# mratsim/laser

Hardware: NVIDIA H100
Metric: sgemm_tflops_m8192_n8192_k8192 (higher is better)
Workload: dtype f32

## Files before the change

### laser_b200/csrc/capi.cu

```cuda
#include "../../include/laser_b200.h"

#include <cuda.h>
#include <cuda_runtime.h>
#include <cudaTypedefs.h>

#include <atomic>
#include <cstdarg>
#include <cstdio>
#include <cstdlib>
#include <cstring>
#include <map>
#include <mutex>
#include <string>
#include <type_traits>
#include <utility>
#include <vector>

#include "gemm_simt.cuh"
#include "gemm_dmma.cuh"
#include "layers.cuh"
#include "split.cuh"
#include "tc_launch.h"

namespace {
// ... 47 lines not shown
  int64_t depth, depth_stride;
  bool operator==(const MapKey &o) const {
    return base == o.base && inner == o.inner && outer == o.outer && stride == o.stride && esz == o.esz &&
           box_inner == o.box_inner && box_outer == o.box_outer && swz == o.swz && depth == o.depth &&
           depth_stride == o.depth_stride;
  }
};
struct MapCacheEntry {
  MapKey key;
  CUtensorMap map;
  bool valid = false;
};
constexpr int kMapCacheSize = 64;

constexpr int kSchedSlots = 256;

struct Ctx {
  MapCacheEntry map_cache[kMapCacheSize];
  int map_cache_next = 0;
  int raster_g = 0;
  bool splitk_enabled = true;
  bool f64_dmma = true;
  bool ring_attr_set = false, dmma_attr_set = false;
  int64_t panel_rows = 1024;
  bool panel_taper = false;
  int kc_faithful = 128;
  bool dyn_sched = true;
  bool pdl = true;
  int64_t batch_ws_bytes = static_cast<int64_t>(1024) << 20;
  bool profiling = false;
  std::vector<EventPair> prof;
  int dev = -1;
  int sm_count = 0;
  cudaStream_t stream = nullptr;
  cudaStream_t up = nullptr, down = nullptr;
  std::vector<cudaEvent_t> panel_ev;
  PFN_cuTensorMapEncodeTiled_v12000 encode = nullptr;
  Buffer ws[4];
  Buffer gather[2];
  Buffer stage[3];
  Buffer splitk;
  Buffer bpanels;
  Buffer layer_ws;
  Buffer tfilt;
  Buffer f16s;
  Buffer sched;
  int sched_next = 0;
  cudaEvent_t ws_free = nullptr;
  std::mutex mu;
  std::mutex host_mu;
  std::mutex tfilt_mu;
  std::atomic<bool> ready{false};
};

constexpr int kMaxDevices = 32;
Ctx g_ctx[kMaxDevices];
std::mutex g_ctx_mu;

int parse_f32_mode(const char *mode) {
  if (!mode) return kDefaultF32Mode;
  if (!strcmp(mode, "f16x3")) return LASER_B200_PATH_F16X3;
  else if (!strcmp(mode, "tf32x3")) return LASER_B200_PATH_TF32X3;
  else if (!strcmp(mode, "tf32x1")) return LASER_B200_PATH_TF32X1;
  else if (!strcmp(mode, "simt")) return LASER_B200_PATH_SIMT;
  return kDefaultF32Mode;
}

int get_ctx(Ctx **out) {
  int dev = 0;
  cudaError_t e = cudaGetDevice(&dev);
  if (e != cudaSuccess) {
    cudaGetLastError();
    return set_error(LASER_B200_ENODEVICE, "no CUDA device: %s", cudaGetErrorString(e));
  }
  if (dev < 0 || dev >= kMaxDevices) return set_error(LASER_B200_ENODEVICE, "device index %d", dev);
  Ctx &c = g_ctx[dev];
  if (!c.ready) {
    std::lock_guard<std::mutex> lk(g_ctx_mu);
    if (!c.ready) {
      cudaDeviceProp prop;
      CUDA_TRY(cudaGetDeviceProperties(&prop, dev));
      if (prop.major != 9 || prop.minor != 0)
        return set_error(LASER_B200_ENODEVICE,
                         "device %d is sm_%d%d; this library is built for sm_90a only (no fallback)",
                         dev, prop.major, prop.minor);
      c.dev = dev;
      c.sm_count = prop.multiProcessorCount;
      CUDA_TRY(cudaStreamCreateWithFlags(&c.stream, cudaStreamNonBlocking));
      CUDA_TRY(cudaStreamCreateWithFlags(&c.up, cudaStreamNonBlocking));
      CUDA_TRY(cudaStreamCreateWithFlags(&c.down, cudaStreamNonBlocking));
      CUDA_TRY(cudaEventCreateWithFlags(&c.ws_free, cudaEventDisableTiming));
      void *fn = nullptr;
      cudaDriverEntryPointQueryResult qres;
      CUDA_TRY(cudaGetDriverEntryPoint("cuTensorMapEncodeTiled", &fn, cudaEnableDefault, &qres));
      if (!fn || qres != cudaDriverEntryPointSuccess)
        return set_error(LASER_B200_ECUDA, "cuTensorMapEncodeTiled not available from the driver");
      c.encode = reinterpret_cast<PFN_cuTensorMapEncodeTiled_v12000>(fn);
      CUDA_TRY(cudaMalloc(&c.sched.ptr, kSchedSlots * 2 * sizeof(unsigned int)));
      c.sched.bytes = kSchedSlots * 2 * sizeof(unsigned int);
      CUDA_TRY(cudaMemset(c.sched.ptr, 0, c.sched.bytes));
      if (const char *kc = getenv("LASER_B200_KC")) {
        const int v = atoi(kc);
        if (v >= 32) c.kc_faithful = v;
      }
      if (const char *rg = getenv("LASER_B200_RASTER")) c.raster_g = atoi(rg);
      if (const char *sk = getenv("LASER_B200_SPLITK")) c.splitk_enabled = atoi(sk) != 0;
      if (const char *dm = getenv("LASER_B200_F64_DMMA")) c.f64_dmma = atoi(dm) != 0;
      if (const char *pt = getenv("LASER_B200_PANEL_TAPER")) c.panel_taper = atoi(pt) != 0;
      if (const char *ds = getenv("LASER_B200_DYNSCHED")) c.dyn_sched = atoi(ds) != 0;
      if (const char *pd = getenv("LASER_B200_PDL")) c.pdl = atoi(pd) != 0;
      if (const char *bw = getenv("LASER_B200_BATCH_WS_MB")) {
        const int64_t v = atoll(bw);
        if (v >= 1) c.batch_ws_bytes = v << 20;
      }
      if (const char *pr = getenv("LASER_B200_PANEL_ROWS")) {
        const int64_t v = atoll(pr) / 256 * 256;
        if (v >= 256) c.panel_rows = v;
      }
      if (g_f32_mode.load() < 0) g_f32_mode.store(parse_f32_mode(getenv("LASER_B200_F32_MODE")));
      c.ready = true;
// ... 484 lines not shown
  return path == LASER_B200_PATH_TF32X1 ? TC_TF32X1 : path == LASER_B200_PATH_TF32X3 ? TC_TF32X3 : TC_F16X3;
}
inline SplitMode split_mode(TcKind k) { return k == TC_TF32X3 ? SPLIT_TF32 : k == TC_F16X3 ? SPLIT_F16X2 : SPLIT_NONE; }

struct BatchArgs {
  int64_t batch, C, bias = 0;
};

template <typename OutT>
int tc_run(Ctx &c, TcKind kind, int64_t M, int64_t N, int64_t K, float alpha, const OperandMaps &ma,
           const OperandMaps &mb, float beta, OutT *C, int64_t rsC, int64_t csC, cudaStream_t s,
           const Epilogue &epi, const F16Scales *f16 = nullptr, bool after_prep = false, const BatchArgs *bat = nullptr,
           int64_t period_a = 1, int64_t period_b = 1) {
  TcLaunch l;
  l.a0 = ma.p0; l.a1 = ma.p1; l.b0 = mb.p0; l.b1 = mb.p1;
  l.a_mn = ma.mn_major; l.b_mn = mb.mn_major;
  l.pdl = c.pdl && after_prep;
  l.dev = c.dev; l.sm_count = c.sm_count; l.stream = s;
  TcParams &p = l.p;
  p.M = M; p.N = N; p.K = K; p.alpha = alpha; p.beta = beta;
  p.C = C; p.rsC = rsC; p.csC = csC; p.epi = epi;
  if (f16) { p.amax_a = f16->a; p.amax_b = f16->b; }
  if (bat) {
    l.batched = true;
    p.batch = static_cast<int>(bat->batch);
    p.period_a = static_cast<int>(period_a);
    p.period_b = static_cast<int>(period_b);
    p.bsC = bat->C;
    p.amax_bs_a = M;
    p.amax_bs_b = N;
    p.bias_bs = bat->bias;
  }
  const int npass = (kind == TC_TF32X3 || kind == TC_F16X3) ? 3 : 1;
  const TcPlanCfg cfg{c.kc_faithful, c.raster_g, c.splitk_enabled, c.sm_count};
  if (kind == TC_BF16 || kind == TC_F16X3) tc_plan<2, std::is_same<OutT, float>::value>(p, npass, cfg);
  else tc_plan<4, std::is_same<OutT, float>::value>(p, npass, cfg);
  if (c.dyn_sched) {
    p.sched = static_cast<unsigned int *>(c.sched.ptr) + 2 * c.sched_next;
    c.sched_next = (c.sched_next + 1) % kSchedSlots;
  }
  auto launch = [&](const TcLaunch &q) -> int {
    int e;
    switch (kind) {
      case TC_TF32X1: e = launch_tc_tf32x1(q); break;
      case TC_TF32X3: e = launch_tc_tf32x3(q); break;
      case TC_BF16: e = launch_tc_bf16(q); break;
      default: e = launch_tc_f16x3(q); break;
    }
    COUNT_LAUNCH();
    if (e != 0) {
      cudaGetLastError();
      return set_error(e == static_cast<int>(cudaErrorMemoryAllocation) ? LASER_B200_ENOMEM : LASER_B200_ECUDA,
                       "tensor-core kernel launch failed: %s", cudaGetErrorString(static_cast<cudaError_t>(e)));
    }
    CHECK_LAUNCH();
    return LASER_B200_OK;
  };
  ProfBracket prof;
  int rc = prof.open(c, s, 0);
  if (rc) return rc;
  if (p.k_splits > 1) {
    if constexpr (std::is_same<OutT, float>::value) {
      const int64_t ws_floats = tc_split_ws_floats(p);
      if ((rc = ensure(c.splitk, static_cast<size_t>(ws_floats) * sizeof(float)))) return rc;
      p.split_ws = static_cast<float *>(c.splitk.ptr);
      if ((rc = launch(l))) return rc;
      const int n_tail = p.num_m_blocks * p.num_n_blocks * p.batch - p.n_direct;
// ... 1297 lines not shown
```

### laser_b200/csrc/gemm_tc.cuh

```cuda
#pragma once

#include <type_traits>

#include "f16_scale.cuh"
#include "ptx.cuh"
#include "tc_params.h"

namespace lb200 {

#ifndef LB200_HOST_EMULATION
static __device__ __noinline__ float epi_act(float v, int act) {
#else
inline float epi_act(float v, int act) {
#endif
  if (act == 1) return fmaxf(v, 0.0f);
  if (act == 2) return tanhf(v);
  if (act == 3) return 1.0f / (1.0f + expf(-v));
  return v;
}

__device__ __forceinline__ float bf16_bits_to_f32(uint16_t h) {
  return __uint_as_float(static_cast<uint32_t>(h) << 16);
}
__device__ __forceinline__ uint16_t f32_to_bf16_bits(float f) {
  uint32_t u = __float_as_uint(f);
  if ((u & 0x7fffffffu) > 0x7f800000u) return static_cast<uint16_t>((u >> 16) | 0x40);
  u += 0x7fffu + ((u >> 16) & 1u);
  return static_cast<uint16_t>(u >> 16);
}

template <int ESZ, uint32_t FMT16, int NPASS, bool A_MN, bool B_MN, typename OutT, bool SCALED, bool BATCHED>
__global__ void __launch_bounds__(TC_THREADS, 1)
gemm_tc_kernel(const __grid_constant__ CUtensorMap mapA0, const __grid_constant__ CUtensorMap mapA1,
               const __grid_constant__ CUtensorMap mapB0, const __grid_constant__ CUtensorMap mapB1,
               const TcParams p) {
  static_assert(NPASS == 1 || NPASS == 3, "one pass, or the three passes of a two-piece product");
  static_assert(ESZ == 2 || (!A_MN && !B_MN), "wgmma reads tf32 operands K-major only (capi.cu transposes MN-major fp32)");
  using Cfg = TcCfg<NPASS>;
  constexpr int STAGES = Cfg::STAGES;
  constexpr int BLOCK_K = TC_ROW_BYTES / ESZ;
  const int sched_id = static_cast<int>(blockIdx.x);
  const int sched_stride = static_cast<int>(gridDim.x);

  LB200_DYN_SMEM(uint8_t, smem_raw);
  uint8_t *smem = reinterpret_cast<uint8_t *>((reinterpret_cast<uintptr_t>(smem_raw) + 1023) &
                                              ~static_cast<uintptr_t>(1023));
  uint64_t *bars = reinterpret_cast<uint64_t *>(smem + STAGES * Cfg::STAGE_BYTES);
  uint64_t *full_bar = bars;
  uint64_t *empty_bar = bars + STAGES;
  uint64_t *sched_full = bars + 2 * STAGES;
  uint64_t *sched_empty = sched_full + 1;
  int *sched_unit = reinterpret_cast<int *>(sched_empty + 1);

  const int warp_idx = threadIdx.x >> 5;
  const int lane = threadIdx.x & 31;
  const int tiles_pp = p.num_m_blocks * p.num_n_blocks;
  const int num_tiles = BATCHED ? tiles_pp * p.batch : tiles_pp;
  const int num_kb = static_cast<int>((p.K + BLOCK_K - 1) / BLOCK_K);
  const int num_units = p.n_direct + (num_tiles - p.n_direct) * p.k_splits;
  auto decode_unit = [&](int u, int &t, int &sp, int &kb_lo, int &kb_hi) {
    if (u < p.n_direct) {
      t = u; sp = -1; kb_lo = 0; kb_hi = num_kb;
    } else {
      const int v = u - p.n_direct;
      const int i = v / p.k_splits;
      t = p.n_direct + i;
      sp = v - i * p.k_splits;
      kb_lo = min(num_kb, sp * p.kb_per_split);
      kb_hi = min(num_kb, kb_lo + p.kb_per_split);
    }
  };
  constexpr int SCHED_CONSUMERS = 1 + TC_EPI_WARPS;
  auto next_unit = [&](uint32_t &ph) -> int {
    ptx::mbar_wait(sched_full, ph);
    const int u = *reinterpret_cast<volatile int *>(sched_unit);
    ptx::mbar_arrive(sched_empty);
    ph ^= 1u;
    return u;
  };

  if (threadIdx.x == 0) {
    ptx::prefetch_tensormap(&mapA0);
    ptx::prefetch_tensormap(&mapB0);
    if constexpr (NPASS == 3) {
      ptx::prefetch_tensormap(&mapA1);
      ptx::prefetch_tensormap(&mapB1);
    }
  }
  if (threadIdx.x == 32) {
    for (int i = 0; i < STAGES; ++i) {
      ptx::mbar_init(&full_bar[i], 1);
      ptx::mbar_init(&empty_bar[i], TC_EPI_WARPS);
    }
    ptx::mbar_init(sched_full, 1);
    ptx::mbar_init(sched_empty, SCHED_CONSUMERS);
    ptx::fence_barrier_init();
  }
  __syncthreads();
  ptx::griddep_wait();

  if (warp_idx < 4) {
    ptx::setmaxnreg_dec<TC_REGS_CTRL>();
    if (warp_idx == 3 && lane == 0) {
      uint32_t phase = 0;
      int next_static = sched_id;
      for (;;) {
        ptx::mbar_wait(sched_empty, phase ^ 1);
        int u;
        if (p.sched) {
          u = static_cast<int>(atomicAdd(p.sched, 1u));
        } else {
          u = next_static;
          next_static += sched_stride;
        }
        if (u >= num_units) u = -1;
        *reinterpret_cast<volatile int *>(sched_unit) = u;
        ptx::mbar_arrive(sched_full);
        phase ^= 1u;
        if (u < 0) {
          if (p.sched) {
            __threadfence();
            if (atomicAdd(p.sched + 1, 1u) == static_cast<unsigned int>(sched_stride - 1)) {
              p.sched[0] = 0u;
              p.sched[1] = 0u;
              __threadfence();
            }
          }
          break;
        }
      }
    } else if (warp_idx == 0 && lane == 0) {
      int stage = 0;
      uint32_t phase = 0, sched_phase = 0;
      constexpr int MN_ATOM = TC_ROW_BYTES / ESZ;
      constexpr int MN_BOX_BYTES = BLOCK_K * TC_ROW_BYTES;
      auto load_a = [&](uint8_t *dst, const CUtensorMap *m, uint64_t *bar, int m0, int k0, int z) {
        if constexpr (!A_MN) {
          if constexpr (BATCHED) ptx::tma_load_3d(dst, m, bar, k0, m0, z);
          else ptx::tma_load_2d(dst, m, bar, k0, m0);
        } else {
#pragma unroll
          for (int c = 0; c < TC_BLOCK_M / MN_ATOM; ++c) {
            if constexpr (BATCHED) ptx::tma_load_3d(dst + c * MN_BOX_BYTES, m, bar, m0 + c * MN_ATOM, k0, z);
            else ptx::tma_load_2d(dst + c * MN_BOX_BYTES, m, bar, m0 + c * MN_ATOM, k0);
          }
        }
      };
      auto load_b = [&](uint8_t *dst, const CUtensorMap *m, uint64_t *bar, int n0, int k0, int z) {
        if constexpr (!B_MN) {
          if constexpr (BATCHED) ptx::tma_load_3d(dst, m, bar, k0, n0, z);
          else ptx::tma_load_2d(dst, m, bar, k0, n0);
        } else {
#pragma unroll
          for (int c = 0; c < TC_BLOCK_N / MN_ATOM; ++c) {
            if constexpr (BATCHED) ptx::tma_load_3d(dst + c * MN_BOX_BYTES, m, bar, n0 + c * MN_ATOM, k0, z);
            else ptx::tma_load_2d(dst + c * MN_BOX_BYTES, m, bar, n0 + c * MN_ATOM, k0);
          }
        }
      };
      for (;;) {
        const int u = next_unit(sched_phase);
        if (u < 0) break;
        int t, sp, mb, nb, kb_lo, kb_hi;
        decode_unit(u, t, sp, kb_lo, kb_hi);
        int za = 0, zb = 0;
        if constexpr (BATCHED) {
          const int bz = t / tiles_pp;
          t -= bz * tiles_pp;
          za = bz % p.period_a;
          zb = bz % p.period_b;
        }
        tile_coords(t, p.num_m_blocks, p.num_n_blocks, p.raster_g, mb, nb);
        const int m0 = mb * TC_BLOCK_M;
        const int n0 = nb * TC_BLOCK_N;
        for (int kb = kb_lo; kb < kb_hi; ++kb) {
          ptx::mbar_wait(&empty_bar[stage], phase ^ 1);
          ptx::mbar_arrive_expect_tx(&full_bar[stage], Cfg::STAGE_BYTES);
          uint8_t *sa = smem + stage * Cfg::STAGE_BYTES;
          uint8_t *sb = sa + Cfg::A_STAGE_BYTES;
          const int k0 = kb * BLOCK_K;
          load_a(sa, &mapA0, &full_bar[stage], m0, k0, za);
          if constexpr (NPASS == 3) load_a(sa + TC_A_TILE_BYTES, &mapA1, &full_bar[stage], m0, k0, za);
          load_b(sb, &mapB0, &full_bar[stage], n0, k0, zb);
          if constexpr (NPASS == 3) load_b(sb + Cfg::B_TILE_BYTES, &mapB1, &full_bar[stage], n0, k0, zb);
          if (++stage == STAGES) { stage = 0; phase ^= 1; }
        }
      }
    }
  } else {
    ptx::setmaxnreg_inc<TC_REGS_EPI>();
    const int g = (warp_idx - 4) >> 2;
    const int wq = warp_idx & 3;
    const int lr = lane >> 2;
    const int lc = 2 * (lane & 3);
    constexpr int MMA_K = 32 / ESZ;
    constexpr int K_STEPS = BLOCK_K / MMA_K;
    constexpr int MN_BOX_BYTES = BLOCK_K * TC_ROW_BYTES;
    constexpr uint32_t A_WG_BYTES = 64 * TC_ROW_BYTES;
    int stage = 0;
    uint32_t phase = 0, sched_phase = 0;
    const bool vec_ok_c = (p.csC == 1) && ((p.rsC & 1) == 0) && ((reinterpret_cast<uintptr_t>(p.C) & (2 * sizeof(OutT) - 1)) == 0) &&
                          (!BATCHED || (p.bsC & 1) == 0);
    float acc[TC_ACC_REGS];
#pragma unroll
    for (int j = 0; j < TC_ACC_REGS; ++j) acc[j] = 0.0f;
    for (;;) {
      int u = 0;
      if (lane == 0) u = next_unit(sched_phase);
      u = __shfl_sync(0xffffffffu, u, 0);
      if (u < 0) break;
      int t, sp, mb, nb, kb_lo, kb_hi;
      decode_unit(u, t, sp, kb_lo, kb_hi);
      int bz = 0, za = 0, zb = 0;
      if constexpr (BATCHED) {
        bz = t / tiles_pp;
        za = bz % p.period_a;
        zb = bz % p.period_b;
        int tl = t - bz * tiles_pp;
        tile_coords(tl, p.num_m_blocks, p.num_n_blocks, p.raster_g, mb, nb);
      } else {
        tile_coords(t, p.num_m_blocks, p.num_n_blocks, p.raster_g, mb, nb);
      }
      const int num_blocks = (kb_hi - kb_lo + p.kb_per_block - 1) / p.kb_per_block;
      const int r_tile = 64 * g + 16 * wq + lr;
      const int64_t row0 = static_cast<int64_t>(mb) * TC_BLOCK_M + r_tile;
      const int64_t col0 = static_cast<int64_t>(nb) * TC_BLOCK_N + lc;
      const bool split_unit = sp >= 0;
      uint32_t amax_row[2] = {0u, 0u}, amax_col[2 * TC_BLOCK_N / 8];
      if constexpr (SCALED) {
#pragma unroll
        for (int h = 0; h < 2; ++h)
          if (row0 + 8 * h < p.M) amax_row[h] = p.amax_a[(BATCHED ? za * p.amax_bs_a : 0) + row0 + 8 * h];
#pragma unroll
        for (int j = 0; j < 2 * TC_BLOCK_N / 8; ++j) {
          const int64_t c = col0 + 8 * (j >> 1) + (j & 1);
          amax_col[j] = c < p.N ? p.amax_b[(BATCHED ? zb * p.amax_bs_b : 0) + c] : 0u;
        }
      }
      float run[TC_ACC_REGS];
#pragma unroll
      for (int j = 0; j < TC_ACC_REGS; ++j) run[j] = 0.0f;
      for (int blk = 0; blk < num_blocks; ++blk) {
        const int kb0 = kb_lo + blk * p.kb_per_block;
        const int kb1 = min(kb_hi, kb0 + p.kb_per_block);
        int prev_stage = -1;
        for (int kb = kb0; kb < kb1; ++kb) {
          ptx::mbar_wait(&full_bar[stage], phase);
          ptx::wgmma_fence();
          const uint32_t a_addr = ptx::smem_u32(smem + stage * Cfg::STAGE_BYTES) + g * A_WG_BYTES;
          const uint32_t b_addr = ptx::smem_u32(smem + stage * Cfg::STAGE_BYTES + Cfg::A_STAGE_BYTES);
#pragma unroll
          for (int pass = 0; pass < NPASS; ++pass) {
            const uint32_t a_tile = a_addr + ((NPASS == 3 && pass == 1) ? TC_A_TILE_BYTES : 0);
            const uint32_t b_tile = b_addr + ((NPASS == 3 && pass == 0) ? Cfg::B_TILE_BYTES : 0);
#pragma unroll
            for (int k = 0; k < K_STEPS; ++k) {
              const uint64_t ad = A_MN ? ptx::make_smem_desc(a_tile + k * MMA_K * TC_ROW_BYTES, MN_BOX_BYTES, 1024, ptx::kLayoutSw128)
                                       : ptx::make_smem_desc(a_tile + k * 32, 0, 1024, ptx::kLayoutSw128);
              const uint64_t bd = B_MN ? ptx::make_smem_desc(b_tile + k * MMA_K * TC_ROW_BYTES, MN_BOX_BYTES, 1024, ptx::kLayoutSw128)
                                       : ptx::make_smem_desc(b_tile + k * 32, 0, 1024, ptx::kLayoutSw128);
              const uint32_t accum = (kb == kb0 && pass == 0 && k == 0) ? 0u : 1u;
              if constexpr (ESZ == 4) ptx::wgmma_m64n128k8_tf32(acc, ad, bd, accum);
              else if constexpr (FMT16 == ptx::kFmtF16) ptx::wgmma_m64n128k16_f16<A_MN ? 1 : 0, B_MN ? 1 : 0>(acc, ad, bd, accum);
              else ptx::wgmma_m64n128k16_bf16<A_MN ? 1 : 0, B_MN ? 1 : 0>(acc, ad, bd, accum);
            }
          }
          ptx::wgmma_commit();
          ptx::wgmma_wait<1>();
          if (prev_stage >= 0 && lane == 0) ptx::mbar_arrive(&empty_bar[prev_stage]);
          prev_stage = stage;
          if (++stage == STAGES) { stage = 0; phase ^= 1; }
        }
        ptx::wgmma_wait<0>();
        ptx::wgmma_hold(acc);
        if (prev_stage >= 0 && lane == 0) ptx::mbar_arrive(&empty_bar[prev_stage]);
#pragma unroll
        for (int j = 0; j < TC_ACC_REGS; ++j) run[j] = __fadd_rn(run[j], acc[j]);
      }
      float alpha_r[2] = {split_unit ? 1.0f : p.alpha, split_unit ? 1.0f : p.alpha};
      if constexpr (SCALED) {
#pragma unroll
        for (int h = 0; h < 2; ++h) alpha_r[h] *= f16x2_unscale(amax_row[h]);
      }
      const float beta_u = split_unit ? 0.0f : p.beta;
      const bool has_epi = !split_unit && ((p.epi.bias != nullptr) || (p.epi.act != 0));
      float *ws_base = nullptr;
      if (split_unit) {
        const int64_t plane = static_cast<int64_t>(sp) * (num_tiles - p.n_direct) + (t - p.n_direct);
        ws_base = p.split_ws + (plane * TC_BLOCK_M + r_tile) * TC_BLOCK_N + lc;
      }
#pragma unroll
      for (int h = 0; h < 2; ++h) {
        const int64_t row = row0 + 8 * h;
        if (!split_unit && row >= p.M) continue;
        const float row_bias =
            (has_epi && p.epi.bias && p.epi.bias_per_row) ? p.epi.bias[(BATCHED ? za * p.bias_bs : 0) + row] : 0.0f;
        OutT *crow = split_unit ? nullptr : reinterpret_cast<OutT *>(p.C) + (BATCHED ? bz * p.bsC : 0) + row * p.rsC;
#pragma unroll
        for (int i = 0; i < TC_BLOCK_N / 8; ++i) {
          float v[2];
#pragma unroll
          for (int e = 0; e < 2; ++e) {
            v[e] = alpha_r[h] * run[4 * i + 2 * h + e];
            if constexpr (SCALED) v[e] *= f16x2_unscale(amax_col[2 * i + e]);
          }
          if (split_unit) {
            *reinterpret_cast<float2 *>(ws_base + 8 * h * TC_BLOCK_N + 8 * i) = make_float2(v[0], v[1]);
            continue;
          }
          const int64_t c = col0 + 8 * i;
          if (c >= p.N) continue;
          const bool pair_ok = vec_ok_c && c + 1 < p.N;
          OutT *dst = crow + c * p.csC;
          if (beta_u != 0.0f) {
            float o[2] = {0.0f, 0.0f};
            if constexpr (sizeof(OutT) == 4) {
              if (pair_ok) { const float2 w = *reinterpret_cast<const float2 *>(dst); o[0] = w.x; o[1] = w.y; }
              else { o[0] = dst[0]; if (c + 1 < p.N) o[1] = dst[p.csC]; }
            } else {
              o[0] = bf16_bits_to_f32(dst[0]);
              if (c + 1 < p.N) o[1] = bf16_bits_to_f32(dst[pair_ok ? 1 : p.csC]);
            }
#pragma unroll
            for (int e = 0; e < 2; ++e) v[e] = fmaf(beta_u, o[e], v[e]);
          }
          if (has_epi) {
#pragma unroll
            for (int e = 0; e < 2; ++e) {
              const float bv = (p.epi.bias && !p.epi.bias_per_row) ? (c + e < p.N ? p.epi.bias[c + e] : 0.0f) : row_bias;
              v[e] = epi_act(v[e] + bv, p.epi.act);
            }
          }
          if constexpr (sizeof(OutT) == 4) {
            if (pair_ok) *reinterpret_cast<float2 *>(dst) = make_float2(v[0], v[1]);
            else { dst[0] = v[0]; if (c + 1 < p.N) dst[p.csC] = v[1]; }
          } else {
            if (pair_ok) *reinterpret_cast<uint32_t *>(dst) = f32_to_bf16_bits(v[0]) | (static_cast<uint32_t>(f32_to_bf16_bits(v[1])) << 16);
            else { dst[0] = f32_to_bf16_bits(v[0]); if (c + 1 < p.N) dst[p.csC] = f32_to_bf16_bits(v[1]); }
          }
        }
      }
    }
  }

  __syncthreads();
}

}
```

### laser_b200/csrc/ptx.cuh

```cuda
#pragma once

#include <cuda.h>
#include <cuda_runtime.h>
#include <stdint.h>

#ifdef LB200_HOST_EMULATION
#include "ptx_emu.h"
#else

#define LB200_DYN_SMEM(T, name) extern __shared__ T name[]

namespace lb200 {
namespace ptx {

__device__ __forceinline__ uint32_t smem_u32(const void *p) {
  return static_cast<uint32_t>(__cvta_generic_to_shared(p));
}

__device__ __forceinline__ bool elect_one() {
  uint32_t pred = 0;
  asm volatile(
      "{\n\t"
      ".reg .pred P;\n\t"
      "elect.sync _|P, 0xffffffff;\n\t"
      "selp.u32 %0, 1, 0, P;\n\t"
      "}\n"
      : "=r"(pred));
  return pred != 0;
}

__device__ __forceinline__ void mbar_init(uint64_t *bar, uint32_t count) {
  asm volatile("mbarrier.init.shared::cta.b64 [%0], %1;" ::"r"(smem_u32(bar)), "r"(count));
}
__device__ __forceinline__ void fence_barrier_init() {
  asm volatile("fence.mbarrier_init.release.cluster;" ::: "memory");
}
__device__ __forceinline__ void fence_proxy_async_smem() {
  asm volatile("fence.proxy.async.shared::cta;" ::: "memory");
}
__device__ __forceinline__ void mbar_arrive_expect_tx(uint64_t *bar, uint32_t bytes) {
// ... 107 lines not shown
      "setp.ne.b32 p, %66, 0;\n\t"
      "wgmma.mma_async.sync.aligned.m64n128k16.f32.bf16.bf16 "
      "{%0, %1, %2, %3, %4, %5, %6, %7, %8, %9, %10, %11, %12, %13, %14, %15, %16, %17, %18, %19, %20, %21, %22, %23, %24, %25, %26, %27, %28, %29, %30, %31, %32, %33, %34, %35, %36, %37, %38, %39, %40, %41, %42, %43, %44, %45, %46, %47, %48, %49, %50, %51, %52, %53, %54, %55, %56, %57, %58, %59, %60, %61, %62, %63}, "
      "%64, %65, p, 1, 1, %67, %68;\n\t"
      "}\n"
      : "+f"(d[0]), "+f"(d[1]), "+f"(d[2]), "+f"(d[3]), "+f"(d[4]), "+f"(d[5]), "+f"(d[6]), "+f"(d[7]),
        "+f"(d[8]), "+f"(d[9]), "+f"(d[10]), "+f"(d[11]), "+f"(d[12]), "+f"(d[13]), "+f"(d[14]), "+f"(d[15]),
        "+f"(d[16]), "+f"(d[17]), "+f"(d[18]), "+f"(d[19]), "+f"(d[20]), "+f"(d[21]), "+f"(d[22]), "+f"(d[23]),
        "+f"(d[24]), "+f"(d[25]), "+f"(d[26]), "+f"(d[27]), "+f"(d[28]), "+f"(d[29]), "+f"(d[30]), "+f"(d[31]),
        "+f"(d[32]), "+f"(d[33]), "+f"(d[34]), "+f"(d[35]), "+f"(d[36]), "+f"(d[37]), "+f"(d[38]), "+f"(d[39]),
        "+f"(d[40]), "+f"(d[41]), "+f"(d[42]), "+f"(d[43]), "+f"(d[44]), "+f"(d[45]), "+f"(d[46]), "+f"(d[47]),
        "+f"(d[48]), "+f"(d[49]), "+f"(d[50]), "+f"(d[51]), "+f"(d[52]), "+f"(d[53]), "+f"(d[54]), "+f"(d[55]),
        "+f"(d[56]), "+f"(d[57]), "+f"(d[58]), "+f"(d[59]), "+f"(d[60]), "+f"(d[61]), "+f"(d[62]), "+f"(d[63])
      : "l"(a_desc), "l"(b_desc), "r"(scale_d), "n"(TA), "n"(TB));
}
__device__ __forceinline__ void wgmma_m64n128k8_tf32(float (&d)[64], uint64_t a_desc, uint64_t b_desc, uint32_t scale_d) {
  asm volatile(
      "{\n\t"
      ".reg .pred p;\n\t"
      "setp.ne.b32 p, %66, 0;\n\t"
      "wgmma.mma_async.sync.aligned.m64n128k8.f32.tf32.tf32 "
      "{%0, %1, %2, %3, %4, %5, %6, %7, %8, %9, %10, %11, %12, %13, %14, %15, %16, %17, %18, %19, %20, %21, %22, %23, %24, %25, %26, %27, %28, %29, %30, %31, %32, %33, %34, %35, %36, %37, %38, %39, %40, %41, %42, %43, %44, %45, %46, %47, %48, %49, %50, %51, %52, %53, %54, %55, %56, %57, %58, %59, %60, %61, %62, %63}, "
      "%64, %65, p, 1, 1;\n\t"
      "}\n"
      : "+f"(d[0]), "+f"(d[1]), "+f"(d[2]), "+f"(d[3]), "+f"(d[4]), "+f"(d[5]), "+f"(d[6]), "+f"(d[7]),
        "+f"(d[8]), "+f"(d[9]), "+f"(d[10]), "+f"(d[11]), "+f"(d[12]), "+f"(d[13]), "+f"(d[14]), "+f"(d[15]),
        "+f"(d[16]), "+f"(d[17]), "+f"(d[18]), "+f"(d[19]), "+f"(d[20]), "+f"(d[21]), "+f"(d[22]), "+f"(d[23]),
        "+f"(d[24]), "+f"(d[25]), "+f"(d[26]), "+f"(d[27]), "+f"(d[28]), "+f"(d[29]), "+f"(d[30]), "+f"(d[31]),
        "+f"(d[32]), "+f"(d[33]), "+f"(d[34]), "+f"(d[35]), "+f"(d[36]), "+f"(d[37]), "+f"(d[38]), "+f"(d[39]),
        "+f"(d[40]), "+f"(d[41]), "+f"(d[42]), "+f"(d[43]), "+f"(d[44]), "+f"(d[45]), "+f"(d[46]), "+f"(d[47]),
        "+f"(d[48]), "+f"(d[49]), "+f"(d[50]), "+f"(d[51]), "+f"(d[52]), "+f"(d[53]), "+f"(d[54]), "+f"(d[55]),
        "+f"(d[56]), "+f"(d[57]), "+f"(d[58]), "+f"(d[59]), "+f"(d[60]), "+f"(d[61]), "+f"(d[62]), "+f"(d[63])
      : "l"(a_desc), "l"(b_desc), "r"(scale_d));
}

__device__ __forceinline__ void griddep_wait() { asm volatile("griddepcontrol.wait;" ::: "memory"); }
__device__ __forceinline__ void griddep_launch_dependents() { asm volatile("griddepcontrol.launch_dependents;" ::: "memory"); }
constexpr uint32_t kLayoutSw128 = 1;
__device__ __forceinline__ uint64_t make_smem_desc(uint32_t smem_addr, uint32_t lbo_bytes, uint32_t sbo_bytes, uint32_t layout) {
  uint64_t d = 0;
  d |= static_cast<uint64_t>((smem_addr & 0x3FFFF) >> 4);
  d |= static_cast<uint64_t>((lbo_bytes >> 4) & 0x3FFF) << 16;
  d |= static_cast<uint64_t>((sbo_bytes >> 4) & 0x3FFF) << 32;
  d |= static_cast<uint64_t>(layout) << 62;
  return d;
}
constexpr uint32_t kFmtF16 = 0, kFmtBF16 = 1, kFmtTF32 = 2;

}
}

#endif
```

### laser_b200/csrc/tc_launch_impl.cuh

```cuda
#pragma once

#include <atomic>

#include "gemm_tc.cuh"
#include "tc_launch.h"

#ifndef LB200_LAUNCH_EX
#define LB200_LAUNCH_EX cudaLaunchKernelEx
#endif

namespace lb200 {

template <int ESZ, uint32_t FMT16, int NPASS, typename OutT, bool SCALED, bool A_MN, bool B_MN, bool BATCHED>
int launch_tc_one(const TcLaunch &l) {
  using Cfg = TcCfg<NPASS>;
  const int64_t units_total = tc_units(l.p);
  cudaLaunchConfig_t cfg{};
  cfg.gridDim = dim3(static_cast<int>(units_total < l.sm_count ? units_total : l.sm_count));
  cfg.blockDim = dim3(TC_THREADS);
  cfg.dynamicSmemBytes = Cfg::SMEM_BYTES;
  cfg.stream = l.stream;
  cudaLaunchAttribute attr[1];
  if (l.pdl) {
    attr[0].id = cudaLaunchAttributeProgrammaticStreamSerialization;
    attr[0].val.programmaticStreamSerializationAllowed = 1;
    cfg.attrs = attr;
    cfg.numAttrs = 1;
  }
  auto kfn = gemm_tc_kernel<ESZ, FMT16, NPASS, A_MN, B_MN, OutT, SCALED, BATCHED>;
  static std::atomic<uint32_t> attr_set{0};
  if (!(attr_set.load(std::memory_order_acquire) & (1u << l.dev))) {
    const cudaError_t e = cudaFuncSetAttribute(kfn, cudaFuncAttributeMaxDynamicSharedMemorySize, Cfg::SMEM_BYTES);
    if (e != cudaSuccess) return static_cast<int>(e);
    attr_set.fetch_or(1u << l.dev, std::memory_order_release);
  }
  return static_cast<int>(LB200_LAUNCH_EX(&cfg, kfn, l.a0, l.a1, l.b0, l.b1, l.p));
}

template <int ESZ, uint32_t FMT16, int NPASS, typename OutT, bool SCALED>
int launch_tc_family(const TcLaunch &l) {
  if constexpr (ESZ == 4) {
    if (l.a_mn || l.b_mn) return static_cast<int>(cudaErrorNotSupported);
    if (l.batched) return launch_tc_one<ESZ, FMT16, NPASS, OutT, SCALED, false, false, true>(l);
    return launch_tc_one<ESZ, FMT16, NPASS, OutT, SCALED, false, false, false>(l);
  }
#define LB200_MAJORS(BATCHED)                                                                                  \
  do {                                                                                                         \
    if (!l.a_mn && !l.b_mn) return launch_tc_one<ESZ, FMT16, NPASS, OutT, SCALED, false, false, BATCHED>(l);   \
    if (!l.a_mn && l.b_mn) return launch_tc_one<ESZ, FMT16, NPASS, OutT, SCALED, false, true, BATCHED>(l);     \
    if (l.a_mn && !l.b_mn) return launch_tc_one<ESZ, FMT16, NPASS, OutT, SCALED, true, false, BATCHED>(l);     \
    return launch_tc_one<ESZ, FMT16, NPASS, OutT, SCALED, true, true, BATCHED>(l);                             \
  } while (0)
  if constexpr (ESZ == 2) {
    if constexpr (SCALED) {
      if (l.batched) LB200_MAJORS(true);
    }
    if (l.batched) return static_cast<int>(cudaErrorNotSupported);
    LB200_MAJORS(false);
  }
#undef LB200_MAJORS
}

}
```

### laser_b200/csrc/tc_params.h

```cpp
#pragma once

#include <stdint.h>

#if defined(__CUDACC__) || defined(LB200_HOST_EMULATION)
#define LB200_HD __host__ __device__
#else
#define LB200_HD
#endif

namespace lb200 {

constexpr int TC_BLOCK_M = 128;
constexpr int TC_BLOCK_N = 128;
constexpr int TC_ROW_BYTES = 128;
constexpr int TC_A_TILE_BYTES = TC_BLOCK_M * TC_ROW_BYTES;
template <int NPASS> struct TcCfg {
  static constexpr int PIECES = (NPASS == 3) ? 2 : 1;
  static constexpr int B_TILE_BYTES = TC_BLOCK_N * TC_ROW_BYTES;
  static constexpr int A_STAGE_BYTES = PIECES * TC_A_TILE_BYTES;
  static constexpr int B_STAGE_BYTES = PIECES * B_TILE_BYTES;
  static constexpr int STAGE_BYTES = A_STAGE_BYTES + B_STAGE_BYTES;
#ifdef TC_STAGES_OVERRIDE
  static constexpr int STAGES = TC_STAGES_OVERRIDE;
#else
// ... 3 lines not shown
};
constexpr int TC_THREADS = 384;
constexpr int TC_EPI_THREADS = 256;
constexpr int TC_EPI_WARPS = TC_EPI_THREADS / 32;
constexpr int TC_ACC_REGS = 64 * TC_BLOCK_N / 128;
constexpr int TC_REGS_CTRL = 40;
constexpr int TC_REGS_EPI = 232;

struct Epilogue {
  const float *bias = nullptr;
  int bias_per_row = 0;
  int act = 0;
};
struct TcParams {
  int64_t M, N, K;
  float alpha, beta;
  void *C;
  int64_t rsC, csC;
  int kb_per_block;
  int raster_g;
  Epilogue epi;
  int n_direct;
  int k_splits;
  int kb_per_split;
  float *split_ws = nullptr;
  int num_m_blocks, num_n_blocks;
  const uint32_t *amax_a = nullptr, *amax_b = nullptr;
  unsigned int *sched = nullptr;
  int batch = 1;
  int period_a = 1, period_b = 1;
  int64_t bsC = 0;
  int64_t amax_bs_a = 0, amax_bs_b = 0;
  int64_t bias_bs = 0;
};

LB200_HD inline void tile_coords(int t, int num_m, int num_n, int G, int &mb, int &nb) {
  const int per_group = G * num_n;
  const int g = t / per_group;
  const int first_m = g * G;
  const int gsz = (G < num_m - first_m) ? G : (num_m - first_m);
  const int r = t - g * per_group;
  mb = first_m + r % gsz;
  nb = r / gsz;
}

struct TcPlanCfg {
  int kc_faithful;
  int raster_g;
  bool splitk_enabled;
  int sm_count;
  int tail_min_k = 2048;
};
template <int ESZ, bool OUT_F32>
inline void tc_plan(TcParams &p, int npass, const TcPlanCfg &cfg) {
  const int block_k = TC_ROW_BYTES / ESZ;
  const int num_kb = static_cast<int>((p.K + block_k - 1) / block_k);
  {
    const int kc = (npass == 3) ? cfg.kc_faithful : 0;
    p.kb_per_block = (kc > 0) ? (kc + block_k - 1) / block_k : num_kb;
    if (p.kb_per_block < 1) p.kb_per_block = 1;
    if (p.kb_per_block > num_kb) p.kb_per_block = num_kb;
  }
  p.raster_g = cfg.raster_g > 0 ? cfg.raster_g : 16;
  p.num_m_blocks = static_cast<int>((p.M + TC_BLOCK_M - 1) / TC_BLOCK_M);
  p.num_n_blocks = static_cast<int>((p.N + TC_BLOCK_N - 1) / TC_BLOCK_N);
  const int64_t tiles = static_cast<int64_t>(p.num_m_blocks) * p.num_n_blocks * p.batch;
  p.k_splits = 1;
  p.kb_per_split = num_kb;
  p.n_direct = static_cast<int>(tiles);
  p.split_ws = nullptr;
  const int units = cfg.sm_count;
  if constexpr (OUT_F32) {
    const int blocks = (num_kb + p.kb_per_block - 1) / p.kb_per_block;
    const int min_tiles = 512 / block_k;
    const int min_blocks = (min_tiles + p.kb_per_block - 1) / p.kb_per_block;
    const int max_s = blocks / min_blocks < 16 ? blocks / min_blocks : 16;
    const int64_t rem = tiles < units ? tiles : tiles % units;
    int S = rem > 0 ? static_cast<int>(units / rem) : 1;
    if (S > max_s) S = max_s;
    const bool worth = S >= 2 && (tiles < units || p.K >= cfg.tail_min_k);
    if (cfg.splitk_enabled && worth && units > 0) {
      const int blocks_per_split = (blocks + S - 1) / S;
      p.k_splits = (blocks + blocks_per_split - 1) / blocks_per_split;
      p.kb_per_split = blocks_per_split * p.kb_per_block;
      if (p.k_splits >= 2) p.n_direct = static_cast<int>(tiles - rem);
      else { p.k_splits = 1; p.kb_per_split = num_kb; }
    }
  }
}
inline int64_t tc_units(const TcParams &p) {
  const int64_t tiles = static_cast<int64_t>(p.num_m_blocks) * p.num_n_blocks * p.batch;
  return p.n_direct + (tiles - p.n_direct) * p.k_splits;
}
inline int64_t tc_split_ws_floats(const TcParams &p) {
  const int64_t tiles = static_cast<int64_t>(p.num_m_blocks) * p.num_n_blocks * p.batch;
  return (tiles - p.n_direct) * p.k_splits * TC_BLOCK_M * TC_BLOCK_N;
}

}
```

Measured before the change: 214.7.

## Pair CTAs in 2-CTA clusters and multicast shared B tiles via TMA

Launches the tensor-core GEMM kernel with clusters of two CTAs that work on vertically adjacent M tiles sharing the same N block. Each CTA loads the B tile for alternating k-blocks and multicasts it to both CTAs. The scheduler, stage releases and barriers become cluster-wide. This is meant to halve the L2/global traffic for B. In exchange it adds cross-CTA synchronisation, so one slow CTA stalls its partner, and the planner and unit decoding get more complex.

Result: slower. 125.5, median of 6 (-41.5%).

```diff
diff --git a/laser_b200/csrc/capi.cu b/laser_b200/csrc/capi.cu
--- a/laser_b200/csrc/capi.cu
+++ b/laser_b200/csrc/capi.cu
@@ -103,6 +103,7 @@
   std::vector<EventPair> prof;
   int dev = -1;
   int sm_count = 0;
+  bool cluster_launch = false;
   cudaStream_t stream = nullptr;
   cudaStream_t up = nullptr, down = nullptr;
   std::vector<cudaEvent_t> panel_ev;
@@ -157,6 +158,7 @@
                          dev, prop.major, prop.minor);
       c.dev = dev;
       c.sm_count = prop.multiProcessorCount;
+      c.cluster_launch = prop.clusterLaunch != 0;
       CUDA_TRY(cudaStreamCreateWithFlags(&c.stream, cudaStreamNonBlocking));
       CUDA_TRY(cudaStreamCreateWithFlags(&c.up, cudaStreamNonBlocking));
       CUDA_TRY(cudaStreamCreateWithFlags(&c.down, cudaStreamNonBlocking));
@@ -707,7 +709,8 @@
     p.bias_bs = bat->bias;
   }
   const int npass = (kind == TC_TF32X3 || kind == TC_F16X3) ? 3 : 1;
-  const TcPlanCfg cfg{c.kc_faithful, c.raster_g, c.splitk_enabled, c.sm_count};
+  TcPlanCfg cfg{c.kc_faithful, c.raster_g, c.splitk_enabled, c.sm_count};
+  cfg.pairs = c.cluster_launch;
   if (kind == TC_BF16 || kind == TC_F16X3) tc_plan<2, std::is_same<OutT, float>::value>(p, npass, cfg);
   else tc_plan<4, std::is_same<OutT, float>::value>(p, npass, cfg);
   if (c.dyn_sched) {
diff --git a/laser_b200/csrc/gemm_tc.cuh b/laser_b200/csrc/gemm_tc.cuh
--- a/laser_b200/csrc/gemm_tc.cuh
+++ b/laser_b200/csrc/gemm_tc.cuh
@@ -39,8 +39,10 @@
   using Cfg = TcCfg<NPASS>;
   constexpr int STAGES = Cfg::STAGES;
   constexpr int BLOCK_K = TC_ROW_BYTES / ESZ;
-  const int sched_id = static_cast<int>(blockIdx.x);
-  const int sched_stride = static_cast<int>(gridDim.x);
+  const int CL = p.cluster;
+  const uint32_t rank = CL > 1 ? ptx::cluster_ctarank() : 0u;
+  const int sched_id = static_cast<int>(blockIdx.x) / CL;
+  const int sched_stride = static_cast<int>(gridDim.x) / CL;
 
   LB200_DYN_SMEM(uint8_t, smem_raw);
   uint8_t *smem = reinterpret_cast<uint8_t *>((reinterpret_cast<uintptr_t>(smem_raw) + 1023) &
@@ -57,26 +59,53 @@
   const int tiles_pp = p.num_m_blocks * p.num_n_blocks;
   const int num_tiles = BATCHED ? tiles_pp * p.batch : tiles_pp;
   const int num_kb = static_cast<int>((p.K + BLOCK_K - 1) / BLOCK_K);
-  const int num_units = p.n_direct + (num_tiles - p.n_direct) * p.k_splits;
-  auto decode_unit = [&](int u, int &t, int &sp, int &kb_lo, int &kb_hi) {
-    if (u < p.n_direct) {
-      t = u; sp = -1; kb_lo = 0; kb_hi = num_kb;
+  const int unit_m = (p.num_m_blocks + CL - 1) / CL;
+  const int units_pp = unit_m * p.num_n_blocks;
+  const int num_unit_tiles = BATCHED ? units_pp * p.batch : units_pp;
+  const int num_units = p.n_direct_units + (num_unit_tiles - p.n_direct_units) * p.k_splits;
+  auto decode_unit = [&](int u, int &bz, int &mb, int &nb, int &t, int &sp, int &kb_lo, int &kb_hi) {
+    int q;
+    if (u < p.n_direct_units) {
+      q = u; sp = -1; kb_lo = 0; kb_hi = num_kb;
     } else {
-      const int v = u - p.n_direct;
+      const int v = u - p.n_direct_units;
       const int i = v / p.k_splits;
-      t = p.n_direct + i;
+      q = p.n_direct_units + i;
       sp = v - i * p.k_splits;
       kb_lo = min(num_kb, sp * p.kb_per_split);
       kb_hi = min(num_kb, kb_lo + p.kb_per_split);
     }
+    bz = BATCHED ? q / units_pp : 0;
+    tile_coords(q - bz * units_pp, unit_m, p.num_n_blocks, p.raster_g / CL, mb, nb);
+    if (CL == 1) {
+      t = q;
+    } else {
+      mb = CL * mb + static_cast<int>(rank);
+      t = mb < p.num_m_blocks ? bz * tiles_pp + tile_index(mb, nb, p.num_m_blocks, p.num_n_blocks, p.raster_g) : -1;
+    }
   };
   constexpr int SCHED_CONSUMERS = 1 + TC_EPI_WARPS;
   auto next_unit = [&](uint32_t &ph) -> int {
-    ptx::mbar_wait(sched_full, ph);
-    const int u = *reinterpret_cast<volatile int *>(sched_unit);
-    ptx::mbar_arrive(sched_empty);
+    int u;
+    if (CL == 1) {
+      ptx::mbar_wait(sched_full, ph);
+      u = *reinterpret_cast<volatile int *>(sched_unit);
+      ptx::mbar_arrive(sched_empty);
+    } else {
+      ptx::mbar_wait_cluster(sched_full, ph);
+      u = *reinterpret_cast<volatile int *>(sched_unit);
+      ptx::mbar_arrive_cluster(sched_empty, 0);
+    }
     ph ^= 1u;
     return u;
+  };
+  auto release_stage = [&](int s) {
+    if (CL == 1) {
+      ptx::mbar_arrive(&empty_bar[s]);
+    } else {
+      ptx::mbar_arrive_cluster(&empty_bar[s], 0);
+      ptx::mbar_arrive_cluster(&empty_bar[s], 1);
+    }
   };
 
   if (threadIdx.x == 0) {
@@ -90,18 +119,19 @@
   if (threadIdx.x == 32) {
     for (int i = 0; i < STAGES; ++i) {
       ptx::mbar_init(&full_bar[i], 1);
-      ptx::mbar_init(&empty_bar[i], TC_EPI_WARPS);
+      ptx::mbar_init(&empty_bar[i], CL * TC_EPI_WARPS);
     }
     ptx::mbar_init(sched_full, 1);
-    ptx::mbar_init(sched_empty, SCHED_CONSUMERS);
+    ptx::mbar_init(sched_empty, CL * SCHED_CONSUMERS);
     ptx::fence_barrier_init();
   }
-  __syncthreads();
+  if (CL > 1) ptx::cluster_sync();
+  else __syncthreads();
   ptx::griddep_wait();
 
   if (warp_idx < 4) {
     ptx::setmaxnreg_dec<TC_REGS_CTRL>();
-    if (warp_idx == 3 && lane == 0) {
+    if (warp_idx == 3 && lane == 0 && rank == 0) {
       uint32_t phase = 0;
       int next_static = sched_id;
       for (;;) {
@@ -114,8 +144,15 @@
           next_static += sched_stride;
         }
         if (u >= num_units) u = -1;
-        *reinterpret_cast<volatile int *>(sched_unit) = u;
-        ptx::mbar_arrive(sched_full);
+        if (CL == 1) {
+          *reinterpret_cast<volatile int *>(sched_unit) = u;
+          ptx::mbar_arrive(sched_full);
+        } else {
+          for (uint32_t r = 0; r < static_cast<uint32_t>(CL); ++r) {
+            ptx::st_shared_cluster_s32(sched_unit, r, u);
+            ptx::mbar_arrive_cluster(sched_full, r);
+          }
+        }
         phase ^= 1u;
         if (u < 0) {
           if (p.sched) {
@@ -147,30 +184,28 @@
         }
       };
       auto load_b = [&](uint8_t *dst, const CUtensorMap *m, uint64_t *bar, int n0, int k0, int z) {
+        auto box = [&](uint8_t *d, int c0, int c1) {
+          if (CL == 1) {
+            if constexpr (BATCHED) ptx::tma_load_3d(d, m, bar, c0, c1, z);
+            else ptx::tma_load_2d(d, m, bar, c0, c1);
+          } else {
+            if constexpr (BATCHED) ptx::tma_load_3d_multicast(d, m, bar, c0, c1, z, 0x3);
+            else ptx::tma_load_2d_multicast(d, m, bar, c0, c1, 0x3);
+          }
+        };
         if constexpr (!B_MN) {
-          if constexpr (BATCHED) ptx::tma_load_3d(dst, m, bar, k0, n0, z);
-          else ptx::tma_load_2d(dst, m, bar, k0, n0);
+          box(dst, k0, n0);
         } else {
 #pragma unroll
-          for (int c = 0; c < TC_BLOCK_N / MN_ATOM; ++c) {
-            if constexpr (BATCHED) ptx::tma_load_3d(dst + c * MN_BOX_BYTES, m, bar, n0 + c * MN_ATOM, k0, z);
-            else ptx::tma_load_2d(dst + c * MN_BOX_BYTES, m, bar, n0 + c * MN_ATOM, k0);
-          }
+          for (int c = 0; c < TC_BLOCK_N / MN_ATOM; ++c) box(dst + c * MN_BOX_BYTES, n0 + c * MN_ATOM, k0);
         }
       };
       for (;;) {
         const int u = next_unit(sched_phase);
         if (u < 0) break;
-        int t, sp, mb, nb, kb_lo, kb_hi;
-        decode_unit(u, t, sp, kb_lo, kb_hi);
-        int za = 0, zb = 0;
-        if constexpr (BATCHED) {
-          const int bz = t / tiles_pp;
-          t -= bz * tiles_pp;
-          za = bz % p.period_a;
-          zb = bz % p.period_b;
-        }
-        tile_coords(t, p.num_m_blocks, p.num_n_blocks, p.raster_g, mb, nb);
+        int bz, t, sp, mb, nb, kb_lo, kb_hi;
+        decode_unit(u, bz, mb, nb, t, sp, kb_lo, kb_hi);
+        const int za = BATCHED ? bz % p.period_a : 0, zb = BATCHED ? bz % p.period_b : 0;
         const int m0 = mb * TC_BLOCK_M;
         const int n0 = nb * TC_BLOCK_N;
         for (int kb = kb_lo; kb < kb_hi; ++kb) {
@@ -181,8 +216,10 @@
           const int k0 = kb * BLOCK_K;
           load_a(sa, &mapA0, &full_bar[stage], m0, k0, za);
           if constexpr (NPASS == 3) load_a(sa + TC_A_TILE_BYTES, &mapA1, &full_bar[stage], m0, k0, za);
-          load_b(sb, &mapB0, &full_bar[stage], n0, k0, zb);
-          if constexpr (NPASS == 3) load_b(sb + Cfg::B_TILE_BYTES, &mapB1, &full_bar[stage], n0, k0, zb);
+          if (CL == 1 || (kb & 1) == static_cast<int>(rank)) {
+            load_b(sb, &mapB0, &full_bar[stage], n0, k0, zb);
+            if constexpr (NPASS == 3) load_b(sb + Cfg::B_TILE_BYTES, &mapB1, &full_bar[stage], n0, k0, zb);
+          }
           if (++stage == STAGES) { stage = 0; phase ^= 1; }
         }
       }
@@ -209,18 +246,9 @@
       if (lane == 0) u = next_unit(sched_phase);
       u = __shfl_sync(0xffffffffu, u, 0);
       if (u < 0) break;
-      int t, sp, mb, nb, kb_lo, kb_hi;
-      decode_unit(u, t, sp, kb_lo, kb_hi);
-      int bz = 0, za = 0, zb = 0;
-      if constexpr (BATCHED) {
-        bz = t / tiles_pp;
-        za = bz % p.period_a;
-        zb = bz % p.period_b;
-        int tl = t - bz * tiles_pp;
-        tile_coords(tl, p.num_m_blocks, p.num_n_blocks, p.raster_g, mb, nb);
-      } else {
-        tile_coords(t, p.num_m_blocks, p.num_n_blocks, p.raster_g, mb, nb);
-      }
+      int bz, t, sp, mb, nb, kb_lo, kb_hi;
+      decode_unit(u, bz, mb, nb, t, sp, kb_lo, kb_hi);
+      const int za = BATCHED ? bz % p.period_a : 0, zb = BATCHED ? bz % p.period_b : 0;
       const int num_blocks = (kb_hi - kb_lo + p.kb_per_block - 1) / p.kb_per_block;
       const int r_tile = 64 * g + 16 * wq + lr;
       const int64_t row0 = static_cast<int64_t>(mb) * TC_BLOCK_M + r_tile;
@@ -267,13 +295,13 @@
           }
           ptx::wgmma_commit();
           ptx::wgmma_wait<1>();
-          if (prev_stage >= 0 && lane == 0) ptx::mbar_arrive(&empty_bar[prev_stage]);
+          if (prev_stage >= 0 && lane == 0) release_stage(prev_stage);
           prev_stage = stage;
           if (++stage == STAGES) { stage = 0; phase ^= 1; }
         }
         ptx::wgmma_wait<0>();
         ptx::wgmma_hold(acc);
-        if (prev_stage >= 0 && lane == 0) ptx::mbar_arrive(&empty_bar[prev_stage]);
+        if (prev_stage >= 0 && lane == 0) release_stage(prev_stage);
 #pragma unroll
         for (int j = 0; j < TC_ACC_REGS; ++j) run[j] = __fadd_rn(run[j], acc[j]);
       }
@@ -284,6 +312,7 @@
       }
       const float beta_u = split_unit ? 0.0f : p.beta;
       const bool has_epi = !split_unit && ((p.epi.bias != nullptr) || (p.epi.act != 0));
+      if (t < 0) continue;
       float *ws_base = nullptr;
       if (split_unit) {
         const int64_t plane = static_cast<int64_t>(sp) * (num_tiles - p.n_direct) + (t - p.n_direct);
@@ -343,7 +372,8 @@
     }
   }
 
-  __syncthreads();
-}
-
-}
+  if (CL > 1) ptx::cluster_sync();
+  else __syncthreads();
+}
+
+}
diff --git a/laser_b200/csrc/ptx.cuh b/laser_b200/csrc/ptx.cuh
--- a/laser_b200/csrc/ptx.cuh
+++ b/laser_b200/csrc/ptx.cuh
@@ -6,6 +6,7 @@
 
 #ifdef LB200_HOST_EMULATION
 #include "ptx_emu.h"
+#include "ptx_cluster_emu.h"
 #else
 
 #define LB200_DYN_SMEM(T, name) extern __shared__ T name[]
@@ -179,6 +180,61 @@
         "+f"(d[48]), "+f"(d[49]), "+f"(d[50]), "+f"(d[51]), "+f"(d[52]), "+f"(d[53]), "+f"(d[54]), "+f"(d[55]),
         "+f"(d[56]), "+f"(d[57]), "+f"(d[58]), "+f"(d[59]), "+f"(d[60]), "+f"(d[61]), "+f"(d[62]), "+f"(d[63])
       : "l"(a_desc), "l"(b_desc), "r"(scale_d));
+}
+
+__device__ __forceinline__ uint32_t cluster_ctarank() {
+  uint32_t r;
+  asm volatile("mov.u32 %0, %%cluster_ctarank;" : "=r"(r));
+  return r;
+}
+__device__ __forceinline__ void cluster_arrive() { asm volatile("barrier.cluster.arrive.release.aligned;" ::: "memory"); }
+__device__ __forceinline__ void cluster_wait() { asm volatile("barrier.cluster.wait.acquire.aligned;" ::: "memory"); }
+__device__ __forceinline__ void cluster_sync() {
+  cluster_arrive();
+  cluster_wait();
+}
+__device__ __forceinline__ uint32_t mapa(const void *p, uint32_t rank) {
+  uint32_t r;
+  asm volatile("mapa.shared::cluster.u32 %0, %1, %2;" : "=r"(r) : "r"(smem_u32(p)), "r"(rank));
+  return r;
+}
+__device__ __forceinline__ void mbar_arrive_cluster(uint64_t *bar, uint32_t rank) {
+  asm volatile("mbarrier.arrive.release.cluster.shared::cluster.b64 _, [%0];" ::"r"(mapa(bar, rank)) : "memory");
+}
+__device__ __forceinline__ void mbar_wait_cluster(uint64_t *bar, uint32_t parity) {
+  uint32_t ok;
+  do {
+    asm volatile(
+        "{\n\t"
+        ".reg .pred P;\n\t"
+        "mbarrier.try_wait.parity.acquire.cluster.shared::cta.b64 P, [%1], %2;\n\t"
+        "selp.u32 %0, 1, 0, P;\n\t"
+        "}\n"
+        : "=r"(ok)
+        : "r"(smem_u32(bar)), "r"(parity)
+        : "memory");
+  } while (!ok);
+}
+__device__ __forceinline__ void st_shared_cluster_s32(int *p, uint32_t rank, int v) {
+  asm volatile("st.shared::cluster.s32 [%0], %1;" ::"r"(mapa(p, rank)), "r"(v) : "memory");
+}
+__device__ __forceinline__ void tma_load_2d_multicast(void *smem_dst, const CUtensorMap *map, uint64_t *bar, int32_t c0,
+                                                      int32_t c1, uint16_t cta_mask) {
+  asm volatile(
+      "cp.async.bulk.tensor.2d.shared::cluster.global.mbarrier::complete_tx::bytes.multicast::cluster"
+      " [%0], [%1, {%3, %4}], [%2], %5;"
+      ::"r"(smem_u32(smem_dst)), "l"(reinterpret_cast<uint64_t>(map)), "r"(smem_u32(bar)),
+        "r"(c0), "r"(c1), "h"(cta_mask)
+      : "memory");
+}
+__device__ __forceinline__ void tma_load_3d_multicast(void *smem_dst, const CUtensorMap *map, uint64_t *bar, int32_t c0,
+                                                      int32_t c1, int32_t c2, uint16_t cta_mask) {
+  asm volatile(
+      "cp.async.bulk.tensor.3d.shared::cluster.global.mbarrier::complete_tx::bytes.multicast::cluster"
+      " [%0], [%1, {%3, %4, %5}], [%2], %6;"
+      ::"r"(smem_u32(smem_dst)), "l"(reinterpret_cast<uint64_t>(map)), "r"(smem_u32(bar)),
+        "r"(c0), "r"(c1), "r"(c2), "h"(cta_mask)
+      : "memory");
 }
 
 __device__ __forceinline__ void griddep_wait() { asm volatile("griddepcontrol.wait;" ::: "memory"); }
diff --git a/laser_b200/csrc/tc_launch_impl.cuh b/laser_b200/csrc/tc_launch_impl.cuh
--- a/laser_b200/csrc/tc_launch_impl.cuh
+++ b/laser_b200/csrc/tc_launch_impl.cuh
@@ -15,17 +15,24 @@
 int launch_tc_one(const TcLaunch &l) {
   using Cfg = TcCfg<NPASS>;
   const int64_t units_total = tc_units(l.p);
+  const int cl = l.p.cluster;
   cudaLaunchConfig_t cfg{};
-  cfg.gridDim = dim3(static_cast<int>(units_total < l.sm_count ? units_total : l.sm_count));
   cfg.blockDim = dim3(TC_THREADS);
   cfg.dynamicSmemBytes = Cfg::SMEM_BYTES;
   cfg.stream = l.stream;
-  cudaLaunchAttribute attr[1];
+  cudaLaunchAttribute attr[2];
+  cfg.attrs = attr;
+  if (cl > 1) {
+    attr[cfg.numAttrs].id = cudaLaunchAttributeClusterDimension;
+    attr[cfg.numAttrs].val.clusterDim.x = static_cast<unsigned>(cl);
+    attr[cfg.numAttrs].val.clusterDim.y = 1;
+    attr[cfg.numAttrs].val.clusterDim.z = 1;
+    ++cfg.numAttrs;
+  }
   if (l.pdl) {
-    attr[0].id = cudaLaunchAttributeProgrammaticStreamSerialization;
-    attr[0].val.programmaticStreamSerializationAllowed = 1;
-    cfg.attrs = attr;
-    cfg.numAttrs = 1;
+    attr[cfg.numAttrs].id = cudaLaunchAttributeProgrammaticStreamSerialization;
+    attr[cfg.numAttrs].val.programmaticStreamSerializationAllowed = 1;
+    ++cfg.numAttrs;
   }
   auto kfn = gemm_tc_kernel<ESZ, FMT16, NPASS, A_MN, B_MN, OutT, SCALED, BATCHED>;
   static std::atomic<uint32_t> attr_set{0};
@@ -34,6 +41,23 @@
     if (e != cudaSuccess) return static_cast<int>(e);
     attr_set.fetch_or(1u << l.dev, std::memory_order_release);
   }
+  int resident = l.sm_count;
+  if (cl > 1) {
+    static std::atomic<int> pairs_resident[32];
+    resident = l.dev < 32 ? pairs_resident[l.dev].load(std::memory_order_relaxed) : 0;
+    if (resident == 0) {
+#ifdef LB200_HOST_EMULATION
+      return static_cast<int>(cudaErrorNotSupported);
+#else
+      cfg.gridDim = dim3(cl);
+      const cudaError_t e = cudaOccupancyMaxActiveClusters(&resident, kfn, &cfg);
+      if (e != cudaSuccess) return static_cast<int>(e);
+#endif
+      if (resident < 1) return static_cast<int>(cudaErrorInvalidConfiguration);
+      if (l.dev < 32) pairs_resident[l.dev].store(resident, std::memory_order_relaxed);
+    }
+  }
+  cfg.gridDim = dim3(cl * static_cast<int>(units_total < resident ? units_total : resident));
   return static_cast<int>(LB200_LAUNCH_EX(&cfg, kfn, l.a0, l.a1, l.b0, l.b1, l.p));
 }
 
diff --git a/laser_b200/csrc/tc_params.h b/laser_b200/csrc/tc_params.h
--- a/laser_b200/csrc/tc_params.h
+++ b/laser_b200/csrc/tc_params.h
@@ -59,6 +59,8 @@
   int64_t bsC = 0;
   int64_t amax_bs_a = 0, amax_bs_b = 0;
   int64_t bias_bs = 0;
+  int cluster = 1;
+  int n_direct_units = 0;
 };
 
 LB200_HD inline void tile_coords(int t, int num_m, int num_n, int G, int &mb, int &nb) {
@@ -71,12 +73,20 @@
   nb = r / gsz;
 }
 
+LB200_HD inline int tile_index(int mb, int nb, int num_m, int num_n, int G) {
+  const int g = mb / G;
+  const int first_m = g * G;
+  const int gsz = (G < num_m - first_m) ? G : (num_m - first_m);
+  return g * G * num_n + nb * gsz + (mb - first_m);
+}
+
 struct TcPlanCfg {
   int kc_faithful;
   int raster_g;
   bool splitk_enabled;
   int sm_count;
   int tail_min_k = 2048;
+  bool pairs = false;
 };
 template <int ESZ, bool OUT_F32>
 inline void tc_plan(TcParams &p, int npass, const TcPlanCfg &cfg) {
@@ -114,10 +124,28 @@
       else { p.k_splits = 1; p.kb_per_split = num_kb; }
     }
   }
+  p.cluster = 1;
+  p.n_direct_units = p.n_direct;
+  if (cfg.pairs && p.num_m_blocks >= 2 && p.raster_g % 2 == 0 && cfg.sm_count >= 2) {
+    const int64_t tiles_pp = static_cast<int64_t>(p.num_m_blocks) * p.num_n_blocks;
+    const int64_t b = p.n_direct / tiles_pp;
+    const int loc = static_cast<int>(p.n_direct - b * tiles_pp);
+    const int G = p.raster_g;
+    const int g = loc / (G * p.num_n_blocks);
+    const int gsz = (G < p.num_m_blocks - g * G) ? G : (p.num_m_blocks - g * G);
+    const int r = loc - g * G * p.num_n_blocks;
+    const int nb = r / gsz, j = r - nb * gsz;
+    if (j % 2 == 0) {
+      const int64_t pairs_pp = static_cast<int64_t>((p.num_m_blocks + 1) / 2) * p.num_n_blocks;
+      p.cluster = 2;
+      p.n_direct_units = static_cast<int>(b * pairs_pp + static_cast<int64_t>(g) * (G / 2) * p.num_n_blocks +
+                                          nb * ((gsz + 1) / 2) + j / 2);
+    }
+  }
 }
 inline int64_t tc_units(const TcParams &p) {
-  const int64_t tiles = static_cast<int64_t>(p.num_m_blocks) * p.num_n_blocks * p.batch;
-  return p.n_direct + (tiles - p.n_direct) * p.k_splits;
+  const int64_t unit_tiles = static_cast<int64_t>((p.num_m_blocks + p.cluster - 1) / p.cluster) * p.num_n_blocks * p.batch;
+  return p.n_direct_units + (unit_tiles - p.n_direct_units) * p.k_splits;
 }
 inline int64_t tc_split_ws_floats(const TcParams &p) {
   const int64_t tiles = static_cast<int64_t>(p.num_m_blocks) * p.num_n_blocks * p.batch;
```
